# BenLangmead/bowtie2

Hardware: AMD Instinct MI355X
Metric: aligned reads/sec (whole node), 150 bp SE vs hg38-like synthetic genome (hg38 unavailable offline), large index (higher is better)
Workload: dtype u8/u64

## Files before the change

bowtie2_amd/csrc/bt2g_align.hpp:

```cpp
#ifndef BT2G_ALIGN_HPP_
#define BT2G_ALIGN_HPP_

#include "bt2g_device.hpp"
#include "../../include/bt2g.h"

namespace bt2g {

#ifdef BT2G_CLASS_MAX_LEN
constexpr int kMaxLen      = BT2G_CLASS_MAX_LEN;
constexpr int kMaxOffs     = BT2G_CLASS_MAX_OFFS;
#else
constexpr int kMaxLen      = 512;
constexpr int kMaxOffs     = 64;
#endif
constexpr int kMaxMm1      = 1024;
constexpr int kMaxRanges   = 2 * kMaxOffs;
constexpr int kMaxSat2     = 4096;
#ifdef BT2G_CLASS_MAX_EDITS
constexpr int kMaxEdits    = BT2G_CLASS_MAX_EDITS;
#else
constexpr int kMaxEdits    = 200;
#endif
#ifdef BT2G_CLASS_MAX_WALK_EDITS
constexpr int kMaxWalkEdits = BT2G_CLASS_MAX_WALK_EDITS;
// ... 219 lines not shown
	uint64_t srow_joff[kMaxSatpos];
	SatPos   sp_view;
	uint32_t lists[kListArena];
	double   masses[kMaxSat2];
	uint8_t  elim[kMaxSat2];
	struct ExtRange { uint32_t off, len, sz; } ex_fw[kMaxRanges * 2], ex_rc[kMaxRanges * 2];
	ExtRange ex_fw2[kMaxRanges * 2], ex_rc2[kMaxRanges * 2];
	DiagIval diags[kMaxDiags];
	int64_t  red_dmin[kMaxAlns], red_dmax[kMaxAlns];
	AlnRes   alns[kMaxAlns];
	BtCand   cands[kMaxCands];
	uint32_t cand_hist[2 * (kMaxLocalScore + 1)];
	uint32_t cand_done[2][kMaxCandDone];
	AlnRes   res;
	BtCand   cands2[kMaxCands];
	BtCand   cands_tmp[kMaxCands];
#ifndef BT2G_NO_PAIRS
	struct MateSave {
		uint32_t len;
		EEHit    exact[2];
		uint32_t n_mm1; uint64_t mm1_elt;
		uint32_t num_offs, nonz_tot, nonz_fw, nonz_rc, n_sranges; uint64_t num_elts;
		uint32_t off_idx2off[kMaxOffs];
		HotHit   hits[2][kMaxOffs];
		EEHit    mm1[kMaxMm1];
		SeedRange sranges[kMaxSat2];
	} ms[2];
	AlnRes   alns_u[2][kMaxAlnsU];
	AlnRes   alns_p[2][kMaxAlns];
	int64_t  redu_dmin[2][kMaxAlnsU], redu_dmax[2][kMaxAlnsU];
	AlnRes   red_anchor[kMaxRedAnchor];
	int64_t  reda_dmin[kMaxRedAnchor], reda_dmax[kMaxRedAnchor];
	AlnRes   ores;
	uint32_t mate_streaks[kMaxSatpos];
#endif
};

BT2_HD uint32_t dp_R(uint32_t rows) {
	const uint32_t r = (rows + 63) / 64;
	return (kMaxLen > 512 && r > 8) ? (r + 7) & ~7u : r;
}
BT2_HD uint64_t dp_cell(uint32_t R, uint32_t i, uint32_t j) {
	const uint32_t l = i / R, r = i % R;
	const uint64_t t = (uint64_t)j + l;
	return (t * R + r) * 64 + l;
}
BT2_HD uint32_t dp_RB(uint32_t rows) { const uint32_t r = (rows + 127) / 128; return r <= 4 ? r : r <= 8 ? 8u : 16u; }
BT2_HD uint64_t dp_cell_pk(uint32_t RB, uint32_t i, uint32_t j) {
	const uint32_t k = i / RB, r = i % RB;
	const uint64_t t = (uint64_t)j + k;
	return (t * RB + r) * 128 + (k >> 6) * 64 + (k & 63);
}
BT2_HD uint64_t dp_pk_cells(uint32_t rows, uint32_t cols) { const uint32_t RB = dp_RB(rows); return ((uint64_t)cols + (rows + RB - 1) / RB) * RB * 128; }


struct DpScratch {
	BT2_G uint32_t* mat;
	BT2_G uint16_t* masks;
	BT2_G uint32_t* pmask;
	BT2_G uint32_t* epoch;
	uint32_t  pmask_words;
};
enum { PB_HD = 1, PB_HE = 2, PB_HF = 4, PB_EO = 8, PB_EE = 16, PB_FO = 32, PB_FE = 64 };
constexpr uint32_t kEpochShift = 13, kEpochMax = (1u << 19) - 1;
constexpr uint32_t kPredTile = 64;
struct EeBand { int32_t lo; uint32_t nd; };
BT2_HD bool ee_band(int rfgapo, int rfgape, uint32_t rows, uint32_t cols, int64_t minsc, EeBand& b) {
	const int64_t budget = -minsc;
	if (budget < 0 || rows == 0 || cols == 0) return false;
	int64_t g;
	if (budget < rfgapo) g = 0; else if (rfgape <= 0) g = rows; else g = (budget - rfgapo) / rfgape + 1;
	if (g > (int64_t)rows - 1) g = (int64_t)rows - 1;
	int64_t dhi = (int64_t)cols - (int64_t)rows + g;
	if (dhi > (int64_t)cols - 1) dhi = (int64_t)cols - 1;
	if (dhi < -g) return false;
	b.lo = (int32_t)g; b.nd = (uint32_t)(dhi + g + 1);
	return true;
}
BT2_HD uint32_t ee_band_rp(uint32_t nd) {
	const uint32_t need = (nd + 127) / 128;
	return need <= 4 ? need : need <= 6 ? 6u : need <= 8 ? 8u : need <= 12 ? 12u : need <= 16 ? 16u : 0u;
}
BT2_HD uint64_t pred_idx(int32_t lo, uint32_t w, uint32_t i, uint32_t j) { return (uint64_t)i * w + (uint32_t)((int32_t)j - (int32_t)i + lo); }
BT2_HD uint64_t pred_at(int32_t lo, uint32_t w, uint32_t i, uint32_t j) { return w ? pred_idx(lo, w, i, j) : dp_cell_pk((uint32_t)lo, i, j); }
BT2_HD uint64_t pred_cells(uint32_t rows, uint32_t cols) { uint32_t rp = ee_band_rp(rows + cols); if (rp == 0) rp = 16; return (uint64_t)rows * rp * 128; }

struct AlState {
	BT2_G Work* wp;
	BT2_HD Work* wp_generic() const { return (Work*)wp; }
	DpScratch dp;
	Rng       rnd;
	int64_t   minsc;
	uint32_t  ridx;
	bool      ext_pre;
	const BT2_G uint32_t* pre_ext_cur;
	const BT2_G uint64_t* pre_joff_cur;
	uint32_t  pf_steps, pf_tiles;
	uint64_t  pf_tile_t;
	uint8_t   m_nofw, m_norc;
	const BT2_G uint8_t* pe_seq[2];
	const BT2_G uint8_t* pe_qual[2];
	uint32_t  pe_len[2];
	ReadParams pe_rp[2];
	int64_t   pe_minsc[2];
	DpScratch dp_main, dp_opp;
	BT2_G BtCand* cands_cur;
	uint32_t  pe_streak;
	uint32_t  pe_pair;
	uint32_t  n_emit;
	int32_t   emit_vmax;
	uint32_t  emit_on;
	uint32_t  max_cols;
	uint32_t  rf_at, ned_at;
	uint32_t  rt_at, rt_bytes, rt_cur;
	uint32_t  wide_cells;
	uint32_t  dyn_bytes;
	uint32_t  fill_rows_done, fill_lastsol, fill_sat8;
};

BT2_HD uint32_t dp_cols_for(const AlignParams& P) { return P.max_dp_cols > kMaxCols ? (uint32_t)(P.max_dp_cols < kMaxColsWide ? P.max_dp_cols : kMaxColsWide) : (uint32_t)kMaxCols; }
BT2_HD uint32_t hot_tail_off(uint32_t max_cols) { return (max_cols + 8 + 15) & ~15u; }
BT2_HD uint32_t hot_tail_bytes(uint32_t max_cols, bool local = true) {
	uint32_t b = (max_cols + 8) * 2;
	if (b < (uint32_t)(kMaxEdits * sizeof(Edit))) b = (uint32_t)(kMaxEdits * sizeof(Edit));
	if (kMaxWalkEdits > kMaxEdits && local && b < (uint32_t)(kMaxWalkEdits * sizeof(Edit))) b = (uint32_t)(kMaxWalkEdits * sizeof(Edit));
	if (local && b < kRadixCntBytes) b = kRadixCntBytes;
	return hot_tail_off(max_cols) + ((b + 15) & ~15u);
}

BT2_HD int comp4(int c) { return c < 4 ? 3 - c : 4; }
BT2_HD int imin(int a, int b) { return a < b ? a : b; }
BT2_HD int imax(int a, int b) { return a > b ? a : b; }
BT2_HD int subs0(int a, int b) { const int r = a - b; return r < 0 ? 0 : r; }

BT2_HD uint8_t code2chr(int c) { return (uint8_t)((0x4E54474341ull >> (8 * (c > 4 ? 4 : c))) & 0xff); }

template <typename SP> BT2_HD int mm_penalty(const SP& P, int q) {
	if (P.mm_type == 3) {
		const int qq = q < 40 ? q : 40;
		const float frac = (float)qq / 40.0f;
		return P.mm_min + (int)(frac * (float)(P.mm_max - P.mm_min));
	}
	if (P.mm_type == 2) return q < 5 ? 0 : (q < 15 ? 10 : (q < 25 ? 20 : 30));
	return P.mm_max;
}

template <typename SP> BT2_HD int sc_score(const SP& P, int rdc, int refm, int q) {
	if (q < 0) q = 0;
	if (q > 255) q = 255;
	if (rdc > 3 || refm > 15) return -P.n_pen;
	if (refm & (1 << rdc)) return P.match_bonus;
	return -mm_penalty(P, q);
}
template <typename SP> BT2_HD int sc_mm(const SP& P, int rdc, int refm, int q) {
	if (q < 0) q = 0;
	if (q > 255) q = 255;
	return (rdc > 3 || refm > 15) ? P.n_pen : mm_penalty(P, q);
}

BT2_HD int max_read_gaps(const AlignParams& P, int64_t minsc, uint32_t rdlen) {
	int64_t sc = (int64_t)rdlen * P.match_bonus;
	bool first = true;
	int num = 0;
	while (sc >= minsc) {
		if (first) { first = false; sc -= P.rdgapo; } else sc -= P.rdgape;
		num++;
	}
	return num - 1;
// ... 33 lines not shown
```

bowtie2_amd/csrc/bt2g_align_kernel.hip:

```cpp
#include <hip/hip_runtime.h>
#include <cstddef>
#include <cstdio>
#include <cstdlib>
#include <new>
#include <type_traits>
#include "bt2g_align_core.hpp"
#include "bt2g_local_pk.hpp"
#include "bt2g_align_kernel.hpp"

namespace bt2g {

__shared__ HotWork g_hot;
__shared__ AlignParams g_P;
__shared__ ReadParams g_rp;
__shared__ PreComp g_pre;
__shared__ AlState g_st;
extern __shared__ __attribute__((aligned(16))) uint8_t g_tail[];
typedef __attribute__((address_space(3))) uint8_t lds_byte;
__device__ __forceinline__ uint32_t lds_addr_of_tail() { return (uint32_t)reinterpret_cast<uintptr_t>((lds_byte*)g_tail); }
__device__ __forceinline__ uint8_t* lds_at(uint32_t a) { return (uint8_t*)reinterpret_cast<lds_byte*>((uintptr_t)(uint32_t)__builtin_amdgcn_readfirstlane((int)a)); }
__device__ __forceinline__ uint8_t* dev_rf() { return lds_at(g_st.rf_at); }
__device__ __forceinline__ int16_t* dev_lastrow() { return reinterpret_cast<int16_t*>(lds_at(g_st.ned_at)); }
__device__ __forceinline__ Edit* dev_ned() { return reinterpret_cast<Edit*>(lds_at(g_st.ned_at)); }
__device__ __forceinline__ uint32_t* dev_rt() { return reinterpret_cast<uint32_t*>(lds_at(g_st.rt_at)); }
alignas(16) __shared__ unsigned char g_ix_raw[sizeof(DevIndex<uint64_t>) > sizeof(DevIndex<uint32_t>) ? sizeof(DevIndex<uint64_t>) : sizeof(DevIndex<uint32_t>)];

__device__ __forceinline__ void wave_fence() { __builtin_amdgcn_fence(__ATOMIC_SEQ_CST, "workgroup"); }

typedef unsigned short u16x2 __attribute__((ext_vector_type(2)));
__device__ __forceinline__ u16x2 p_make(unsigned short lo, unsigned short hi) { u16x2 v; v.x = lo; v.y = hi; return v; }
__device__ __forceinline__ u16x2 p_splat(int v) { return p_make((unsigned short)v, (unsigned short)v); }
__device__ __forceinline__ u16x2 p_subs(u16x2 a, u16x2 b) { return __builtin_elementwise_sub_sat(a, b); }
__device__ __forceinline__ u16x2 p_max(u16x2 a, u16x2 b) { return __builtin_elementwise_max(a, b); }
__device__ __forceinline__ u16x2 p_min(u16x2 a, u16x2 b) { return __builtin_elementwise_min(a, b); }
__device__ __forceinline__ unsigned short s_subs(unsigned short a, unsigned short b) { return __builtin_elementwise_sub_sat(a, b); }
__device__ __forceinline__ unsigned short s_max(unsigned short a, unsigned short b) { return a > b ? a : b; }
__device__ __forceinline__ uint32_t umax32(uint32_t a, uint32_t b) { return a > b ? a : b; }
__device__ __forceinline__ uint32_t p_bits(u16x2 v) { return __builtin_bit_cast(uint32_t, v); }
__device__ __forceinline__ u16x2 p_from(uint32_t v) { return __builtin_bit_cast(u16x2, v); }
__device__ __forceinline__ u16x2 p_ne(u16x2 a, u16x2 b) { return p_from(pk::nz(p_bits(a ^ b))); }
__device__ __forceinline__ uint32_t shift_in(uint32_t lo, uint32_t hi) { return __builtin_amdgcn_alignbit(hi, lo, 16); }
template <int CTRL, int ROW_MASK>
__device__ __forceinline__ uint32_t dpp0(uint32_t v) { return (uint32_t)__builtin_amdgcn_update_dpp(0, (int)v, CTRL, ROW_MASK, 0xf, true); }
constexpr int kDppRowShr = 0x110, kDppWaveShl1 = 0x130, kDppWaveShr1 = 0x138, kDppBcast15 = 0x142, kDppBcast31 = 0x143;

template <int RP, bool PRED, bool W16>
__device__ __forceinline__ int fill_ee_u8_band(const AlignParams& P, bool fw, uint32_t rows, uint32_t cols, int lo, int thr, uint8_t* __restrict__ pm, uint32_t& rows_done) {
	constexpr uint32_t kBias = W16 ? 0xffffu : 0xffu;
	constexpr int kLastLo = W16 ? -32768 : -0xff;
	rows_done = rows;
	constexpr int N2 = 2 * RP;
	constexpr uint32_t W = 128u * RP;
	const int lane = threadIdx.x & 63;
	const int dd0 = lane * N2;
	const int j00 = dd0 - lo;
	uint32_t refS[RP];
	u16x2 Hp[RP], Fp[RP];
#pragma unroll
	for (int k = 0; k < RP; k++) {
		uint32_t sel = 0, h = 0;
#pragma unroll
		for (int hh = 0; hh < 2; hh++) {
			const int j = j00 + 2 * k + hh;
			const bool real = (uint32_t)j < cols;
			const uint32_t code = real ? (uint32_t)__builtin_ctz((uint32_t)dev_rf()[real ? j : 0] | 16u) : 4u;
			sel |= (code | 0x0c00u) << (16 * hh);
			h |= (real ? kBias : 0u) << (16 * hh);
		}
		refS[k] = sel; Hp[k] = p_from(h); Fp[k] = p_splat(0);
	}
	if (PRED) for (uint32_t j = (uint32_t)lane; j < cols; j += 64) dev_lastrow()[j] = (int16_t)kLastLo;
	const int rdgape = __builtin_amdgcn_readfirstlane(P.rdgape), rdgapo = __builtin_amdgcn_readfirstlane(P.rdgapo), gapbar = __builtin_amdgcn_readfirstlane(P.gapbar);
	const u16x2 rdoP = p_splat(rdgapo), rfoP = p_splat(__builtin_amdgcn_readfirstlane(P.rfgapo)), rfeP = p_splat(__builtin_amdgcn_readfirstlane(P.rfgape));
	uint32_t npen_word = (uint32_t)__builtin_amdgcn_readfirstlane(P.n_pen) & 0xffu;
	uint32_t k7f = 0x007f007fu;
	asm("" : "+v"(npen_word), "+v"(k7f));
	const int jin63 = 64 * N2 - lo;
	auto cap = [](uint32_t v) -> unsigned short { constexpr uint32_t m = W16 ? 0xffffu : 1023u; return (unsigned short)(v > m ? m : v); };
	const uint32_t D = (uint32_t)N2 * (uint32_t)rdgape;
	const uint32_t lD = (uint32_t)lane * D, lDprev = lane ? lD - D : 0u;
	u16x2 decP[RP];
#pragma unroll
	for (int k = 0; k < RP; k++) decP[k] = p_make(cap((uint32_t)(2 * k) * (uint32_t)rdgape), cap((uint32_t)(2 * k + 1) * (uint32_t)rdgape));
	u16x2 HP[RP];
#pragma unroll
	for (int k = 0; k < RP; k++) HP[k] = p_splat(0);
	for (uint32_t c0 = 0; c0 < rows; c0 += 64) {
		uint32_t tab = 0;
		{
			const uint32_t ri = c0 + (uint32_t)lane;
			if (ri < rows) {
				const int c = rd_char(g_hot, g_hot.len, fw, ri);
				const int q = rd_qual(g_hot, g_hot.len, fw, ri) - 33;
				const uint32_t mm = (uint32_t)(c > 3 ? P.n_pen : mm_penalty(P, q < 0 ? 0 : q)) & 0xffu;
				tab = mm * 0x01010101u;
				if (c <= 3) tab &= ~(0xffu << (8 * c));
			}
		}
		uint32_t chq;
		{
			int jc = jin63 + (int)c0 + lane; jc = jc < 0 ? 0 : jc; if (jc > (int)cols) jc = (int)cols;
			chq = (uint32_t)__builtin_ctz((uint32_t)dev_rf()[jc] | 16u) | 0x0c00u;
		}
		const uint32_t nrow = (uint32_t)__builtin_amdgcn_readfirstlane((int)(rows - c0 < 64u ? rows - c0 : 64u));
		for (uint32_t ii = 0; ii < nrow; ii++) {
			const uint32_t i = c0 + ii;
			const uint32_t T1 = (uint32_t)__builtin_amdgcn_readlane((int)tab, (int)ii);
			const bool bar = (int)i < gapbar || (int)(rows - i - 1) < gapbar;
			const bool nof = bar || i == 0;
			const uint32_t nxtH = dpp0<kDppWaveShl1, 0xf>(p_bits(Hp[0])), nxtF = dpp0<kDppWaveShl1, 0xf>(p_bits(Fp[0]));
			u16x2 penP[RP], HupP[RP], FupP[RP], fP[RP], HdP[RP];
#pragma unroll
			for (int k = 0; k < RP; k++) {
				penP[k] = p_from(__builtin_amdgcn_perm(npen_word, T1, refS[k]));
				HupP[k] = p_from(shift_in(p_bits(Hp[k]), k + 1 < RP ? p_bits(Hp[k + 1 < RP ? k + 1 : 0]) : nxtH));
				FupP[k] = p_from(shift_in(p_bits(Fp[k]), k + 1 < RP ? p_bits(Fp[k + 1 < RP ? k + 1 : 0]) : nxtF));
				fP[k] = nof ? p_splat(0) : p_max(p_subs(FupP[k], rfeP), p_subs(HupP[k], rfoP));
				HdP[k] = p_max(p_subs(Hp[k], penP[k]), fP[k]);
			}
			u16x2 EP[RP];
			if (!bar) {
				unsigned short e0[N2];
				unsigned short carry = 0;
#pragma unroll
				for (int c = 0; c < N2; c++) {
					const u16x2 u = p_subs(HdP[c >> 1], rdoP);
					e0[c] = carry;
					carry = s_max(s_subs(carry, (unsigned short)rdgape), (c & 1) ? u.y : u.x);
				}
				uint32_t Y = (uint32_t)carry + lD;
				Y = umax32(Y, dpp0<kDppRowShr + 1, 0xf>(Y));
				Y = umax32(Y, dpp0<kDppRowShr + 2, 0xf>(Y));
				Y = umax32(Y, dpp0<kDppRowShr + 4, 0xf>(Y));
				Y = umax32(Y, dpp0<kDppRowShr + 8, 0xf>(Y));
				Y = umax32(Y, dpp0<kDppBcast15, 0xa>(Y));
				Y = umax32(Y, dpp0<kDppBcast31, 0xc>(Y));
				const uint32_t Pprev = dpp0<kDppWaveShr1, 0xf>(Y);
				const u16x2 einP = p_splat((int)(Pprev - lDprev));
#pragma unroll
				for (int k = 0; k < RP; k++) EP[k] = p_max(p_make(e0[2 * k], e0[2 * k + 1]), p_subs(einP, decP[k]));
			} else {
#pragma unroll
				for (int k = 0; k < RP; k++) EP[k] = p_splat(0);
			}
#pragma unroll
			for (int k = 0; k < RP; k++) HP[k] = p_max(HdP[k], EP[k]);
			if (PRED) {
				const uint32_t prvH = dpp0<kDppWaveShr1, 0xf>(p_bits(HP[RP - 1])), prvE = dpp0<kDppWaveShr1, 0xf>(p_bits(EP[RP - 1]));
				const u16x2 rdeP = p_splat(rdgape);
				const uint32_t nogap = bar ? (uint32_t)(PB_HE | PB_HF) * 0x10001u : 0u;
				BT2_G uint8_t* rowp = (BT2_G uint8_t*)pm + (uint64_t)i * W + (uint32_t)dd0;
#pragma unroll
				for (int k = 0; k < RP; k++) {
					const u16x2 hlP = p_from(shift_in(k > 0 ? p_bits(HP[k > 0 ? k - 1 : 0]) : prvH, p_bits(HP[k])));
					const u16x2 elP = p_from(shift_in(k > 0 ? p_bits(EP[k > 0 ? k - 1 : 0]) : prvE, p_bits(EP[k])));
					const u16x2 h = HP[k], e = EP[k], f = fP[k];
					uint32_t n = p_bits(p_ne(f + rfeP, FupP[k]));
					n = pk::shl1_or(n, p_bits(p_ne(f + rfoP, HupP[k])));
					n = pk::shl1_or(n, p_bits(p_ne(e + rdeP, elP)));
					n = pk::shl1_or(n, p_bits(p_ne(e + rdoP, hlP)));
					n = pk::shl1_or(n, p_bits(p_ne(h, f)));
					n = pk::shl1_or(n, p_bits(p_ne(h, e)));
					n = pk::shl1_or(n, p_bits(p_ne(h + penP[k], Hp[k])));
					const uint32_t c = (n | nogap) ^ k7f;
					*reinterpret_cast<BT2_G uint16_t*>(rowp + 2 * k) = (uint16_t)__builtin_amdgcn_perm(0u, c, 0x0c0c0200u);
				}
			}
#pragma unroll
			for (int k = 0; k < RP; k++) { Hp[k] = HP[k]; Fp[k] = fP[k]; }
			if (!PRED && (i & 3u) == 3u) {
				u16x2 m = HP[0];
#pragma unroll
				for (int k = 1; k < RP; k++) m = p_max(m, HP[k]);
				if (!__any((int)s_max(m.x, m.y) >= thr)) { rows_done = i + 1; return 0; }
			}
			{
				uint32_t newel = dpp0<kDppWaveShl1, 0xf>(refS[0]);
				{ const int sq = __builtin_amdgcn_readlane((int)chq, (int)ii); asm("v_writelane_b32 %0, %1, 63" : "+v"(newel) : "s"(sq)); }
#pragma unroll
				for (int k = 0; k < RP; k++) refS[k] = shift_in(refS[k], k + 1 < RP ? refS[k + 1 < RP ? k + 1 : 0] : newel);
			}
		}
	}
	int best = 0;
	const int jl0 = (int)rows - 1 + j00;
#pragma unroll
	for (int k = 0; k < RP; k++) {
#pragma unroll
		for (int hh = 0; hh < 2; hh++) {
			const int j = jl0 + 2 * k + hh;
			const int h = hh ? (int)HP[k].y : (int)HP[k].x;
			if ((uint32_t)j < cols) { best = imax(best, h); if (PRED) dev_lastrow()[j] = (int16_t)imax(h - (int)kBias, kLastLo); }
		}
	}
#pragma unroll
	for (int s = 32; s > 0; s >>= 1) best = imax(best, __shfl_xor(best, s));
	return best;
}

constexpr int kLo = -32768;
__device__ __forceinline__ int subs16(int a, int b) { const int v = a - b; return v < kLo ? kLo : v; }

template <int R>
__device__ __forceinline__ int fill_ee_i16_wave(const AlignParams& P, bool fw, uint32_t rows, uint32_t cols,
                                               uint64_t* __restrict__ scratch) {
	const int lane = threadIdx.x & 63;
	const uint32_t nlanes = (rows + R - 1) / R;
	int rdc[R], mmp[R], veto[R];
#pragma unroll
	for (int r = 0; r < R; r++) {
		const uint32_t i = (uint32_t)lane * R + r;
		const bool valid = i < rows;
		rdc[r] = valid ? rd_char(g_hot, g_hot.len, fw, i) : 4;
		const int q = valid ? rd_qual(g_hot, g_hot.len, fw, i) - 33 : 0;
		mmp[r] = mm_penalty(P, q < 0 ? 0 : q);
		veto[r] = (valid && ((int)i < P.gapbar || (int)(rows - i - 1) < P.gapbar)) ? 1 : 0;
	}
	int Hprev[R], Eprev[R];
#pragma unroll
	for (int r = 0; r < R; r++) { Hprev[r] = kLo; Eprev[r] = kLo; }
	int myHlast = kLo, myFlast = kLo, upHdiag = kLo, refm = 0, best = kLo;
	const uint32_t steps = cols + nlanes - 1;
	const bool lane_has_last = ((rows - 1) / R) == (uint32_t)lane;
	const int last_r = (int)((rows - 1) % R);
	for (uint32_t t = 0; t < steps; t++) {
		const int upH = __shfl_up(myHlast, 1);
		const int upF = __shfl_up(myFlast, 1);
		int upRef = __shfl_up(refm, 1);
		if (lane == 0) upRef = (t < cols) ? dev_rf()[t] : 16;
		refm = upRef;
		const int j = (int)t - lane;
		const bool active = j >= 0 && j < (int)cols && (uint32_t)lane < nlanes;
		int refc = 4;
		if (refm & 1) refc = 0; else if (refm & 2) refc = 1; else if (refm & 4) refc = 2; else if (refm & 8) refc = 3;
		int hdiag = (lane == 0) ? 0x7fff : (j == 0 ? kLo : upHdiag);
		int fin_h = upH, fin_f = upF;
		int Hnew[R], Enew[R], Fnew[R];
#pragma unroll
		for (int r = 0; r < R; r++) {
			int pen;
			if (rdc[r] > 3 || refc > 3) pen = P.n_pen; else pen = (rdc[r] == refc) ? -P.match_bonus : mmp[r];
			const int e = (j == 0) ? kLo : imax(subs16(Eprev[r], P.rdgape), veto[r] ? kLo : subs16(Hprev[r], P.rdgapo));
			int f;
			if (lane == 0 && r == 0) f = kLo;
			else f = veto[r] ? kLo : imax(subs16(fin_f, P.rfgape), subs16(fin_h, P.rfgapo));
			const int h = imax(imax(subs16(hdiag, pen), e), f);
			Hnew[r] = h; Enew[r] = e; Fnew[r] = f;
			hdiag = Hprev[r];
			fin_h = h; fin_f = f;
		}
		if (active) {
			uint64_t* base = scratch + ((uint64_t)t * R) * 64 + lane;
#pragma unroll
			for (int r = 0; r < R; r++) base[r * 64] = (uint64_t)(uint16_t)Hnew[r] | ((uint64_t)(uint16_t)Enew[r] << 16) | ((uint64_t)(uint16_t)Fnew[r] << 32);
#pragma unroll
			for (int r = 0; r < R; r++) { Hprev[r] = Hnew[r]; Eprev[r] = Enew[r]; }
			if (lane_has_last) best = imax(best, Hnew[last_r]);
		}
		upHdiag = upH;
		if (active) { myHlast = Hnew[R - 1]; myFlast = Fnew[R - 1]; }
	}
	return __shfl(best, (int)((rows - 1) / R));
}

// ... 499 lines not shown
		for (int q = 0; q < K; q++) {
			if (__ballot((idx >> 6) == (uint32_t)q) == 0ull) continue;
			const uint32_t g = (uint32_t)__builtin_amdgcn_ds_bpermute((int)((idx & 63u) << 2), (int)v[q]);
			if ((idx >> 6) == (uint32_t)q) r = g;
		}
		return r;
	}
	static __device__ __forceinline__ void flush_samp_rows(BT2_G SampRow* dst, uint32_t lo, uint32_t hi, uint32_t src, uint32_t cnt) {
		const uint32_t l = threadIdx.x & 63;
		if (l < cnt) { SampRow r; r.topf = ((uint64_t)hi << 32) | lo; r.src = src; r.done = 0; gst(dst + l, r); }
	}
	template <typename TOff>
	static __device__ __forceinline__ void resolve_rows(const DevEbwt<TOff>& e, const SampRow* rows, uint32_t n, uint64_t* out) {
		wave_fence();
		const uint32_t lane = threadIdx.x & 63;
		if (lane < n) {
			uint32_t steps = 0;
			const TOff joff = bt2g::get_offset(e, (TOff)rows[lane].topf, steps);
			out[lane] = joff_pack((uint64_t)joff, steps);
		}
		wave_fence();
	}
	static __device__ __forceinline__ bool contains_u32(const uint32_t* p, uint32_t n, uint32_t v) {
		wave_fence();
		const uint32_t lane = threadIdx.x & 63;
		for (uint32_t base = 0; base < n; base += 64) {
			const uint32_t i = base + lane;
			if (__ballot(i < n && gld(p + (i < n ? i : 0)) == v)) return true;
		}
		return false;
	}
	static __device__ __attribute__((noinline)) void unseen_list(const uint32_t* seen_, uint32_t nseen_, uint32_t n_, uint32_t* out_) {
		wave_fence();
		const uint32_t* seen = uni_ptr(seen_); uint32_t* out = uni_ptr(out_);
		const uint32_t nseen = uni(nseen_), n = uni(n_);
		const uint32_t lane = threadIdx.x & 63;
		uint32_t count = 0;
		for (uint32_t p0 = 0; p0 < n; p0 += 2048) {
			uint32_t bm = 0;
			for (uint32_t base = 0; base < nseen; base += 64) {
				const uint32_t mine = base + lane < nseen ? gld(seen + base + lane) : 0xffffffffu;
				const uint32_t cnt = nseen - base < 64u ? nseen - base : 64u;
				for (uint32_t t = 0; t < cnt; t++) {
					const uint32_t v = (uint32_t)__builtin_amdgcn_readlane((int)mine, (int)t) - p0;
					if (v < 2048u && (v >> 5) == lane) bm |= 1u << (v & 31);
				}
			}
			const uint32_t pend = n - p0 < 2048u ? n - p0 : 2048u;
			for (uint32_t b = 0; b < pend; b += 64) {
				const uint32_t j = b + lane;
				const uint32_t word = (uint32_t)__shfl((int)bm, (int)(j >> 5));
				const bool unseen = j < pend && !((word >> (j & 31)) & 1u);
				const unsigned long long m = __ballot(unseen);
				if (unseen) gst(out + count + (uint32_t)__popcll(m & ((1ull << lane) - 1ull)), p0 + j);
				count += (uint32_t)__popcll(m);
			}
		}
		wave_fence();
	}
	static __device__ __forceinline__ void iota_u32(uint32_t* p, uint32_t n) {
		wave_fence();
		for (uint32_t i = threadIdx.x & 63; i < n; i += 64) gst(p + i, i);
		wave_fence();
	}
	static __device__ __forceinline__ void copy_words(void* dst, const void* src, uint32_t nwords) {
		wave_fence();
		const uint32_t* s = reinterpret_cast<const uint32_t*>(src);
		uint32_t* d = reinterpret_cast<uint32_t*>(dst);
		for (uint32_t i = threadIdx.x & 63; i < nwords; i += 64) gst(d + i, gld(s + i));
		wave_fence();
	}
	static __device__ __forceinline__ void set_epoch(uint32_t* p, uint32_t e) { if ((threadIdx.x & 63) == 0) *p = e; wave_fence(); }
	static __device__ __forceinline__ void bt_tile_pred(const DpScratch& dp, int32_t band_lo, uint32_t band_w, uint32_t row, uint32_t col, uint32_t epoch, uint32_t dir,
	                                                    uint32_t& pr, uint32_t& mk) {
		wave_fence();
		const uint32_t d = threadIdx.x & 63;
		uint32_t p = 0, m = 0;
		const uint32_t dr = dir == 1 ? 0u : d, dc = dir == 2 ? 0u : d;
		const uint32_t dd = (uint32_t)((int32_t)col - (int32_t)row + band_lo) + dr - dc;
		const bool ok = dr <= row && dc <= col && (band_w == 0u || dd < band_w);
		if (uni(g_st.rt_cur)) {
			if (ok) {
				const uint32_t r = row - dr, bit = r * band_w + dd;
				p = gld(reinterpret_cast<const uint8_t*>(dp.mat) + (uint64_t)r * band_w + dd);
				m = (dev_rt()[bit >> 5] >> (bit & 31u)) & 1u;
			}
		} else if (ok) {
			const uint64_t idx = pred_at(band_lo, band_w, row - dr, col - dc);
			p = gld(reinterpret_cast<const uint8_t*>(dp.mat) + idx);
			const uint32_t w = gld(dp.pmask + idx);
			m = (w >> kEpochShift) == epoch ? (w & 1u) : 0u;
		}
		pr = p; mk = m;
	}
	static __device__ __forceinline__ bool marks_batchable() { return true; }
	static __device__ __forceinline__ void pred_tile8(const DpScratch& dp, int32_t band_lo, uint32_t band_w, uint32_t epoch, uint32_t row, uint32_t col, uint32_t dir, uint32_t flag,
	                                                  uint32_t& plo, uint32_t& phi, uint32_t& mk) {
		wave_fence();
		const uint8_t* pm = reinterpret_cast<const uint8_t*>(dp.mat);
		const bool chip = uni(g_st.rt_cur) != 0u;
		uint32_t pb[8], mw[8];
#pragma unroll
		for (uint32_t i = 0; i < 8; i++) {
			const uint32_t r = row - (dir == 1u ? 0u : i), c = col - (dir == 2u ? 0u : i);
			const uint32_t dd = (uint32_t)((int32_t)c - (int32_t)r + band_lo);
			const bool ok = flag && (int32_t)r >= 0 && (int32_t)c >= 0 && dd < band_w;
			const uint32_t bit = r * band_w + dd;
			pb[i] = ok ? (uint32_t)gld(pm + (uint64_t)r * band_w + dd) : 0u;
			if (chip) mw[i] = ok ? (dev_rt()[bit >> 5] >> (bit & 31u)) & 1u : 0u;
			else { const uint32_t w = ok ? gld(dp.pmask + (uint64_t)r * band_w + dd) : 0u; mw[i] = (w >> kEpochShift) == epoch ? (w & 1u) : 0u; }
		}
		plo = pb[0] | (pb[1] << 8) | (pb[2] << 16) | (pb[3] << 24);
		phi = pb[4] | (pb[5] << 8) | (pb[6] << 16) | (pb[7] << 24);
		mk = mw[0] | (mw[1] << 1) | (mw[2] << 2) | (mw[3] << 3) | (mw[4] << 4) | (mw[5] << 5) | (mw[6] << 6) | (mw[7] << 7);
	}
	static __device__ __forceinline__ uint32_t marks_of_cells(const DpScratch& dp, int32_t band_lo, uint32_t band_w, uint32_t epoch, uint32_t r, uint32_t c, uint32_t flag) {
		wave_fence();
		const uint32_t dd = (uint32_t)((int32_t)c - (int32_t)r + band_lo);
		const bool ok = flag && (int32_t)r >= 0 && (int32_t)c >= 0 && dd < band_w;
		const uint32_t bit = r * band_w + dd;
		if (uni(g_st.rt_cur)) return ok ? (dev_rt()[bit >> 5] >> (bit & 31u)) & 1u : 0u;
		const uint32_t w = ok ? gld(dp.pmask + (uint64_t)r * band_w + dd) : 0u;
		return (w >> kEpochShift) == epoch ? (w & 1u) : 0u;
	}
	static __device__ __forceinline__ void mark_cells(const DpScratch& dp, int32_t band_lo, uint32_t band_w, uint32_t epoch, uint32_t r, uint32_t c, uint32_t flag) {
		const uint32_t dd = (uint32_t)((int32_t)c - (int32_t)r + band_lo);
		const bool ok = flag && (int32_t)r >= 0 && (int32_t)c >= 0 && dd < band_w;
		const uint32_t bit = r * band_w + dd;
		if (uni(g_st.rt_cur)) { if (ok) __hip_atomic_fetch_or(dev_rt() + (bit >> 5), 1u << (bit & 31u), __ATOMIC_RELAXED, __HIP_MEMORY_SCOPE_WAVEFRONT); }
		else if (ok) gst(dp.pmask + (uint64_t)r * band_w + dd, 1u | (epoch << kEpochShift));
		wave_fence();
	}
	static __device__ __forceinline__ void rt_mark(const DpScratch& dp, int32_t band_lo, uint32_t band_w, uint32_t epoch, uint32_t row, uint32_t col) {
		if (uni(g_st.rt_cur)) {
			const uint32_t bit = row * band_w + (uint32_t)((int32_t)col - (int32_t)row + band_lo);
			if ((threadIdx.x & 63) == 0) __hip_atomic_fetch_or(dev_rt() + (bit >> 5), 1u << (bit & 31u), __ATOMIC_RELAXED, __HIP_MEMORY_SCOPE_WAVEFRONT);
		} else gst(dp.pmask + pred_at(band_lo, band_w, row, col), 1u | (epoch << kEpochShift));
	}
	static __device__ __forceinline__ void rt_mark_lane(const DpScratch& dp, int32_t band_lo, uint32_t band_w, uint32_t epoch, uint32_t r, uint32_t c) {
		if (uni(g_st.rt_cur)) {
			const uint32_t bit = r * band_w + (uint32_t)((int32_t)c - (int32_t)r + band_lo);
			__hip_atomic_fetch_or(dev_rt() + (bit >> 5), 1u << (bit & 31u), __ATOMIC_RELAXED, __HIP_MEMORY_SCOPE_WAVEFRONT);
		} else gst(dp.pmask + pred_at(band_lo, band_w, r, c), 1u | (epoch << kEpochShift));
	}
	static __device__ __forceinline__ void rt_begin(const DpScratch& dp, uint32_t rows, bool band) {
		wave_fence();
		const uint32_t w = band ? uni(gld(dp.epoch + 2)) : 0u;
		const uint32_t rt_bytes = uni(g_st.rt_bytes);
		const bool on = w != 0u && rows * (w >> 3) <= rt_bytes;
		if (on) {
			uint4* q = reinterpret_cast<uint4*>(dev_rt());
			const uint32_t n16 = (rows * (w >> 3) + 15u) >> 4;
			for (uint32_t i = threadIdx.x & 63; i < n16; i += 64) q[i] = make_uint4(0, 0, 0, 0);
		}
		if ((threadIdx.x & 63) == 0) g_st.rt_cur = on ? 1u : 0u;
		wave_fence();
	}
	static __device__ __forceinline__ void load_seed_hits(const bt2g_seed_hit* src_fw, const bt2g_seed_hit* src_rc, uint32_t nseeds, bool skip_fw, bool skip_rc) {
		for (int fwi = 0; fwi < 2; fwi++) {
			const bt2g_seed_hit* src = fwi == 0 ? src_fw : src_rc;
			const bool skip = fwi == 0 ? skip_fw : skip_rc;
			for (uint32_t i = threadIdx.x & 63; i < nseeds; i += 64) {
				HotHit h; h.topf = h.topb = 0; h.size = h.esize = 0;
				if (!skip) {
					const uint64_t topf = gld(&src[i].topf), botf = gld(&src[i].botf);
					if (botf > topf) { h.topf = topf; h.topb = gld(&src[i].topb); h.size = h.esize = (uint32_t)(botf - topf); }
				}
				g_hot.hits[fwi][i] = h;
				g_hot.sorted[fwi][i] = 0;
			}
		}
	}
	static __device__ __forceinline__ uint64_t seed_key(bool fw, uint32_t depth, uint32_t L, bool& ok) {
		const uint32_t k = threadIdx.x & 63;
		uint64_t part = 0;
		bool bad = false;
		if (k < L) {
			const int ch = fw ? (int)g_hot.seq[depth + k] : comp4(g_hot.seq[depth + L - 1 - k]);
			bad = ch > 3;
			part = (uint64_t)(ch & 3) << (2 * (L - 1 - k));
		}
		ok = __ballot(bad) == 0ull;
		uint32_t lo = (uint32_t)part, hi = (uint32_t)(part >> 32);
#pragma unroll
		for (int s = 32; s > 0; s >>= 1) { lo |= (uint32_t)__shfl_xor((int)lo, s); hi |= (uint32_t)__shfl_xor((int)hi, s); }
		return ((uint64_t)hi << 32) | lo;
	}
	static __device__ __forceinline__ uint32_t find_key(const uint64_t* keys, const uint8_t* lens, uint32_t n, uint64_t key, uint8_t len) {
		const uint32_t lane = threadIdx.x & 63;
		for (uint32_t base = 0; base < n; base += 64) {
			const uint32_t i = base + lane;
// ... 682 lines not shown
	};
	if (P.paired) {
#ifdef BT2G_NO_PAIRS
		return hipErrorInvalidValue;
#else
		const uint32_t extra = spare(reinterpret_cast<const void*>(&k_align_pairs<TOff>), tail);
		hipLaunchKernelGGL(k_align_pairs<TOff>, dim3(n_waves), dim3(64), tail + extra, st, ix, P, rd, d_rparams, d_results, result_stride,
		                   d_arena, arena_stride, mat_bytes, mask_bytes, pmask_bytes, d_next, d_prof, pre, max_read_len, max_cols, 0u, extra);
#endif
	} else {
		uint32_t rt_bytes = 0;
		hipFuncAttributes fa{};
		static const bool rt_off = getenv("BT2G_RT_LDS") && atoi(getenv("BT2G_RT_LDS")) == 0;
		if (!rt_off && P.match_bonus == 0 && lds_per_wave != 0 && hipFuncGetAttributes(&fa, reinterpret_cast<const void*>(&k_align_reads<TOff>)) == hipSuccess) {
			const uint64_t used = (uint64_t)fa.sharedSizeBytes + tail;
			const uint32_t want = ((max_read_len ? max_read_len : 1u) * 16u + 15u) & ~15u;
			if (used + want <= lds_per_wave) rt_bytes = want;
		}
		const uint32_t extra = spare(reinterpret_cast<const void*>(&k_align_reads<TOff>), tail + rt_bytes);
		static const bool dbg_occ = getenv("BT2G_DEBUG_OCC") != nullptr;
		if (dbg_occ) {
			int nb = 0;
			(void)hipOccupancyMaxActiveBlocksPerMultiprocessor(&nb, reinterpret_cast<const void*>(&k_align_reads<TOff>), 64, tail + rt_bytes + extra);
			fprintf(stderr, "[bt2g] k_align_reads: %d waves per CU resident (LDS %u static + %u tail + %u marks + %u spare; budget %u per wave), %u waves launched\n",
			        nb, (unsigned)fa.sharedSizeBytes, tail, rt_bytes, extra, lds_per_wave, n_waves);
		}
		hipLaunchKernelGGL(k_align_reads<TOff>, dim3(n_waves), dim3(64), tail + rt_bytes + extra, st, ix, P, rd, d_rparams, d_results, result_stride,
		                   d_arena, arena_stride, mat_bytes, mask_bytes, pmask_bytes, d_next, d_prof, pre, max_read_len, max_cols, rt_bytes, extra);
	}
	return hipGetLastError();
}

__global__ void __launch_bounds__(64) __attribute__((amdgpu_waves_per_eu(BT2G_WAVES_PER_EU, BT2G_WAVES_PER_EU), amdgpu_num_vgpr(BT2G_NUM_VGPR)))
k_dp_fill(AlignParams P, const bt2g_dp_problem* __restrict__ probs, uint32_t n, const uint8_t* __restrict__ d_rd, const uint8_t* __restrict__ d_qu,
          const uint8_t* __restrict__ d_rf, uint8_t* __restrict__ d_out, uint8_t* __restrict__ scratch, uint64_t scratch_stride,
          uint64_t mat_bytes, uint64_t mask_bytes, uint64_t pmask_bytes, uint32_t max_cols) {
	const uint32_t lane = threadIdx.x & 63;
	g_P = P;
	g_st.max_cols = max_cols; g_st.rf_at = lds_addr_of_tail(); g_st.ned_at = g_st.rf_at + hot_tail_off(max_cols);
	g_st.rt_at = 0; g_st.rt_bytes = 0; g_st.rt_cur = 0; g_st.dyn_bytes = 0; g_st.wide_cells = 0;
	DpScratch dp;
	carve_scratch(dp, scratch + (uint64_t)blockIdx.x * scratch_stride, mat_bytes, mask_bytes, pmask_bytes);
	g_st.dp = dp; g_st.wp = (BT2_G Work*)scratch; g_st.emit_on = 0;
	wave_fence();
	for (uint32_t p = blockIdx.x; p < n; p += gridDim.x) {
		const bt2g_dp_problem pr = probs[p];
		const uint32_t rows = pr.rows, cols = pr.cols;
		BT2_G bt2g_dp_out* out = (BT2_G bt2g_dp_out*)(d_out + pr.out_off);
		wave_fence();
		g_hot.len = rows;
		for (uint32_t i = lane; i < rows; i += 64) { g_hot.seq[i] = d_rd[pr.rd_off + i]; g_hot.qual[i] = d_qu[pr.rd_off + i]; }
		for (uint32_t j = lane; j < cols + 1; j += 64) dev_rf()[j] = d_rf[pr.rf_off + j];
		g_hot.n_dp_cells_score = g_hot.n_dp_cells_full = g_hot.n_dp_pass = 0;
		wave_fence();
		int64_t best;
		uint32_t lastsolcol = 0, sat8 = 0;
		if (pr.kind == BT2G_DP_LOCAL) best = DevPlat::dp_fill_local(g_P, *g_st.wp_generic(), true, rows, cols, (uint32_t*)dp.mat, (int64_t)pr.minsc, lastsolcol, sat8);
		else {
			const bool band_form = pr.kind == BT2G_DP_EE_U8 || pr.kind == BT2G_DP_EE_I16_BAND;
			if ((threadIdx.x & 63) == 0) g_st.wide_cells = pr.kind == BT2G_DP_EE_I16 ? 1u : 0u;
			wave_fence();
			best = (pr.kind == BT2G_DP_EE_I16_BAND && !DevPlat::ee_wide_band(rows, cols, (int64_t)pr.minsc)) ? INT64_MIN
			     : DevPlat::dp_fill_ee(g_P, *g_st.wp_generic(), true, rows, cols, dp, pr.kind != BT2G_DP_EE_U8, (int64_t)pr.minsc);
			(void)band_form;
		}
		wave_fence();
		const bool band_kind = pr.kind == BT2G_DP_EE_U8 || pr.kind == BT2G_DP_EE_I16_BAND;
		const bool has_mat = !band_kind || (best != INT64_MIN && best >= (int64_t)pr.minsc);
		const int32_t band_lo = (int32_t)dp.epoch[1];
		const uint32_t band_w = dp.epoch[2];
		if (lane == 0) {
			out->best = best; out->lastsolcol = lastsolcol; out->sat8 = sat8; out->pad = 0;
			out->band_lo = band_kind && has_mat ? band_lo : 0; out->band_w = band_kind && has_mat ? band_w : 0;
			out->has_matrix = has_mat ? 1u : 0u;
		}
		BT2_G uint8_t* body = (BT2_G uint8_t*)(d_out + pr.out_off + sizeof(bt2g_dp_out));
		if (band_kind) {
			const uint32_t c4 = (cols + 3u) & ~3u;
			BT2_G int16_t* lr = (BT2_G int16_t*)body;
			for (uint32_t j = lane; j < c4; j += 64) lr[j] = (has_mat && j < cols) ? dev_lastrow()[j] : (int16_t)(pr.kind == BT2G_DP_EE_U8 ? -0xff : -32768);
			if (has_mat) {
				BT2_G uint8_t* pm = body + (uint64_t)c4 * 2;
				const BT2_G uint8_t* src = (const BT2_G uint8_t*)dp.mat;
				for (uint64_t k = lane; k < (uint64_t)rows * band_w; k += 64) pm[k] = src[k];
			}
		} else if (pr.kind == BT2G_DP_LOCAL) {
			const uint32_t RB = dp_RB(rows);
			const BT2_G uint8_t* src = (const BT2_G uint8_t*)dp.mat;
			const uint64_t ncell = (uint64_t)rows * cols;
			for (uint64_t k = lane; k < ncell; k += 64) body[k] = src[dp_cell_pk(RB, (uint32_t)(k / cols), (uint32_t)(k % cols))];
		} else {
			const uint32_t R = dp_R(rows);
			const BT2_G uint64_t* m64 = (const BT2_G uint64_t*)dp.mat;
			BT2_G int32_t* H = (BT2_G int32_t*)body;
			const uint64_t ncell = (uint64_t)rows * cols;
			for (uint64_t k = lane; k < ncell; k += 64) {
				const uint32_t i = (uint32_t)(k / cols), j = (uint32_t)(k % cols);
				const uint64_t c = m64[dp_cell(R, i, j)];
				const uint32_t h = (uint32_t)(c & 0xffff), e = (uint32_t)((c >> 16) & 0xffff), f = (uint32_t)((c >> 32) & 0xffff);
				if (pr.kind == BT2G_DP_EE_I16) { H[k] = (int32_t)(int16_t)h; H[ncell + k] = (int32_t)(int16_t)e; H[2 * ncell + k] = (int32_t)(int16_t)f; }
				else { H[k] = (int32_t)h; H[ncell + k] = (int32_t)e; H[2 * ncell + k] = (int32_t)f; }
			}
		}
		wave_fence();
	}
}

hipError_t launch_dp_fill(const AlignParams& P, const bt2g_dp_problem* d_probs, uint32_t n, const uint8_t* d_rd, const uint8_t* d_qu, const uint8_t* d_rf,
                          uint8_t* d_out, uint8_t* d_scratch, uint64_t scratch_stride, uint64_t mat_bytes, uint64_t mask_bytes, uint64_t pmask_bytes,
                          uint32_t n_waves, uint32_t max_cols, hipStream_t st) {
	if (n == 0) return hipSuccess;
	hipLaunchKernelGGL(k_dp_fill, dim3(n < n_waves ? n : n_waves), dim3(64), hot_tail_bytes(max_cols), st, P, d_probs, n, d_rd, d_qu, d_rf, d_out, d_scratch, scratch_stride, mat_bytes, mask_bytes, pmask_bytes, max_cols);
	return hipGetLastError();
}

void align_scratch_sizes(uint32_t max_len, bool paired, uint32_t maxhalf, uint32_t max_cols, uint64_t& mat_bytes, uint64_t& mask_bytes, uint64_t& pmask_bytes, uint64_t& arena_stride) {
	const uint32_t rows = max_len ? max_len : 1;
	const uint32_t R = dp_R(rows);
	uint32_t cols = paired ? max_cols + 4 : rows + 4 * maxhalf + 1 + 4;
	if (cols > max_cols + 4) cols = max_cols + 4;
	const uint32_t lanes = (rows + R - 1) / R;
	mat_bytes = (((uint64_t)cols + lanes) * R * 64 * 8 + 255) & ~(uint64_t)255;
	const uint64_t pred_bytes = (pred_cells(rows, cols) + 255) & ~(uint64_t)255;
	if (pred_bytes > mat_bytes) mat_bytes = pred_bytes;
	mask_bytes = ((uint64_t)rows * cols * 2 + 255) & ~(uint64_t)255;
#ifdef BT2G_KCLASS_W5
	mat_bytes = pred_bytes; mask_bytes = 256;
#endif
	const uint64_t wf_cells = ((uint64_t)cols + 128) * dp_RB(rows) * 128;
	const uint64_t mask_cells = pred_cells(rows, cols) > wf_cells ? pred_cells(rows, cols) : wf_cells;
	pmask_bytes = 256 + ((mask_cells * 4 + 255) & ~(uint64_t)255);
	arena_stride = ((sizeof(Work) + 255) & ~(uint64_t)255) + (paired ? 2 : 1) * (mat_bytes + mask_bytes + pmask_bytes);
	arena_stride = (arena_stride + 4095) & ~(uint64_t)4095;
}

uint64_t align_work_bytes() { return sizeof(Work); }
uint32_t align_waves_per_cu() { return 4u * BT2G_WAVES_PER_EU; }

template hipError_t launch_align<uint32_t>(const DevIndex<uint32_t>&, const AlignParams&, const bt2g_reads&, const ReadParams*, uint8_t*, uint64_t, uint8_t*, uint64_t, uint64_t, uint64_t, uint64_t, uint32_t, unsigned int*, unsigned long long*, const PreComp&, uint32_t, uint32_t, uint32_t, hipStream_t);
template hipError_t launch_align<uint64_t>(const DevIndex<uint64_t>&, const AlignParams&, const bt2g_reads&, const ReadParams*, uint8_t*, uint64_t, uint8_t*, uint64_t, uint64_t, uint64_t, uint64_t, uint32_t, unsigned int*, unsigned long long*, const PreComp&, uint32_t, uint32_t, uint32_t, hipStream_t);

}

#define BT2G_CLASS_ENTRIES(PFX) \
extern "C" hipError_t PFX##_launch_align(int off_size, const void* ix, const bt2g_align_params* P, const bt2g_reads* rd, const bt2g_read_params* d_rparams, \
                                         uint8_t* d_results, uint64_t result_stride, uint8_t* d_arena, uint64_t arena_stride, \
                                         uint64_t mat_bytes, uint64_t mask_bytes, uint64_t pmask_bytes, uint32_t n_waves, unsigned int* d_next, unsigned long long* d_prof, \
                                         const void* pre, uint32_t max_read_len, uint32_t max_cols, uint32_t lds_per_wave, hipStream_t st) { \
	using namespace bt2g; \
	const PreComp& pc = *reinterpret_cast<const PreComp*>(pre); \
	return off_size == 4 \
		? launch_align(*reinterpret_cast<const DevIndex<uint32_t>*>(ix), *P, *rd, d_rparams, d_results, result_stride, d_arena, arena_stride, mat_bytes, mask_bytes, pmask_bytes, n_waves, d_next, d_prof, pc, max_read_len, max_cols, lds_per_wave, st) \
		: launch_align(*reinterpret_cast<const DevIndex<uint64_t>*>(ix), *P, *rd, d_rparams, d_results, result_stride, d_arena, arena_stride, mat_bytes, mask_bytes, pmask_bytes, n_waves, d_next, d_prof, pc, max_read_len, max_cols, lds_per_wave, st); \
} \
extern "C" uint32_t PFX##_waves_per_cu(void) { return bt2g::align_waves_per_cu(); } \
 \
extern "C" uint32_t PFX##_static_lds(void) { \
	hipFuncAttributes a32, a64; \
	if (hipFuncGetAttributes(&a32, reinterpret_cast<const void*>(&bt2g::k_align_reads<uint32_t>)) != hipSuccess) return 0xffffffffu; \
	if (hipFuncGetAttributes(&a64, reinterpret_cast<const void*>(&bt2g::k_align_reads<uint64_t>)) != hipSuccess) return 0xffffffffu; \
	return (uint32_t)(a32.sharedSizeBytes > a64.sharedSizeBytes ? a32.sharedSizeBytes : a64.sharedSizeBytes); \
} \
extern "C" uint64_t PFX##_work_bytes(void) { return bt2g::align_work_bytes(); } \
 \
extern "C" uint32_t PFX##_max_len(void) { return (uint32_t)bt2g::kMaxLen; } \
extern "C" uint32_t PFX##_max_offs(void) { return (uint32_t)bt2g::kMaxOffs; } \
extern "C" uint32_t PFX##_max_alns(void) { return (uint32_t)bt2g::kMaxAlns; } \
 \
extern "C" void PFX##_scratch_sizes(uint32_t max_len, int paired, uint32_t maxhalf, uint32_t max_cols, uint64_t* mat_bytes, uint64_t* mask_bytes, uint64_t* pmask_bytes, uint64_t* arena_stride) { \
	bt2g::align_scratch_sizes(max_len, paired != 0, maxhalf, max_cols, *mat_bytes, *mask_bytes, *pmask_bytes, *arena_stride); \
}
#ifdef BT2G_KCLASS_W5
BT2G_CLASS_ENTRIES(bt2g_w5)
#endif
#ifdef BT2G_KCLASS_BK
BT2G_CLASS_ENTRIES(bt2g_bk)
#endif
#ifdef BT2G_KCLASS_LR
BT2G_CLASS_ENTRIES(bt2g_lr)
#endif
```

Before: 6.447 million.

## Block predecessor matrix rows so each lane writes 16-byte vector stores

Changes the banded predecessor-matrix layout so several consecutive rows (RB = 8/4/2 depending on RP) are interleaved into 1 KiB blocks. Each lane accumulates its per-row codes in registers and issues one 16-byte store per block, replacing many 2-byte scattered stores during the DP fill. Readers in the traceback and debug-dump paths switch to the new blocked address function, and the scratch size rounds rows up to a multiple of 8. The cost is extra register shuffling per row, padding stores for partial blocks, and more complex indexing on the traceback loads.

Result: no change. 6.462 million, median of 3 (+0.2%).

```diff
diff --git a/bowtie2_amd/csrc/bt2g_align.hpp b/bowtie2_amd/csrc/bt2g_align.hpp
--- a/bowtie2_amd/csrc/bt2g_align.hpp
+++ b/bowtie2_amd/csrc/bt2g_align.hpp
@@ -325,8 +325,15 @@
 	return need <= 4 ? need : need <= 6 ? 6u : need <= 8 ? 8u : need <= 12 ? 12u : need <= 16 ? 16u : 0u;
 }
 BT2_HD uint64_t pred_idx(int32_t lo, uint32_t w, uint32_t i, uint32_t j) { return (uint64_t)i * w + (uint32_t)((int32_t)j - (int32_t)i + lo); }
+BT2_HD uint32_t pred_band_rb_log2(uint32_t w) { return w == 128u ? 3u : w == 256u ? 2u : w == 512u ? 1u : 0u; }
+BT2_HD uint64_t pred_band_at(uint32_t w, uint32_t i, uint32_t dd) {
+	const uint32_t rbs = pred_band_rb_log2(w), n2s = rbs ? 4u - rbs : 0u;
+	return (uint64_t)(i >> rbs) * (w << rbs) + ((dd >> n2s) << (n2s + rbs)) + ((i & ((1u << rbs) - 1u)) << n2s) + (dd & ((1u << n2s) - 1u));
+}
+BT2_HD uint64_t pred_band_bytes(uint32_t w, uint32_t rows) { return (uint64_t)((rows + 7u) & ~7u) * w; }
 BT2_HD uint64_t pred_at(int32_t lo, uint32_t w, uint32_t i, uint32_t j) { return w ? pred_idx(lo, w, i, j) : dp_cell_pk((uint32_t)lo, i, j); }
 BT2_HD uint64_t pred_cells(uint32_t rows, uint32_t cols) { uint32_t rp = ee_band_rp(rows + cols); if (rp == 0) rp = 16; return (uint64_t)rows * rp * 128; }
+BT2_HD uint64_t pred_band_cells(uint32_t rows, uint32_t cols) { uint32_t rp = ee_band_rp(rows + cols); if (rp == 0) rp = 16; return pred_band_bytes(rp * 128u, rows); }
 
 struct AlState {
 	BT2_G Work* wp;
diff --git a/bowtie2_amd/csrc/bt2g_align_kernel.hip b/bowtie2_amd/csrc/bt2g_align_kernel.hip
--- a/bowtie2_amd/csrc/bt2g_align_kernel.hip
+++ b/bowtie2_amd/csrc/bt2g_align_kernel.hip
@@ -85,6 +85,23 @@
 	u16x2 HP[RP];
 #pragma unroll
 	for (int k = 0; k < RP; k++) HP[k] = p_splat(0);
+	constexpr uint32_t RBS = RP == 1 ? 3u : RP == 2 ? 2u : RP == 4 ? 1u : 0u, RB = 1u << RBS;
+	uint32_t blk[4] = {0u, 0u, 0u, 0u};
+	auto blk_push = [&](const uint32_t* cb) {
+		if constexpr (RP == 1) {
+			blk[0] = shift_in(blk[0], blk[1]); blk[1] = shift_in(blk[1], blk[2]); blk[2] = shift_in(blk[2], blk[3]);
+			blk[3] = __builtin_amdgcn_perm(cb[0], blk[3], 0x06040302u);
+		} else if constexpr (RP == 2) {
+			blk[0] = blk[1]; blk[1] = blk[2]; blk[2] = blk[3]; blk[3] = __builtin_amdgcn_perm(cb[1], cb[0], 0x06040200u);
+		} else if constexpr (RP == 4) {
+			blk[0] = blk[2]; blk[1] = blk[3]; blk[2] = __builtin_amdgcn_perm(cb[1], cb[0], 0x06040200u); blk[3] = __builtin_amdgcn_perm(cb[3], cb[2], 0x06040200u);
+		}
+	};
+	auto blk_store = [&](uint32_t b) {
+		typedef uint32_t u32x4 __attribute__((ext_vector_type(4)));
+		u32x4 v; v.x = blk[0]; v.y = blk[1]; v.z = blk[2]; v.w = blk[3];
+		*reinterpret_cast<BT2_G u32x4*>((BT2_G uint8_t*)pm + ((uint64_t)b << 10) + ((uint32_t)lane << 4)) = v;
+	};
 	for (uint32_t c0 = 0; c0 < rows; c0 += 64) {
 		uint32_t tab = 0;
 		{
@@ -150,6 +167,7 @@
 				const u16x2 rdeP = p_splat(rdgape);
 				const uint32_t nogap = bar ? (uint32_t)(PB_HE | PB_HF) * 0x10001u : 0u;
 				BT2_G uint8_t* rowp = (BT2_G uint8_t*)pm + (uint64_t)i * W + (uint32_t)dd0;
+				uint32_t cb[RP];
 #pragma unroll
 				for (int k = 0; k < RP; k++) {
 					const u16x2 hlP = p_from(shift_in(k > 0 ? p_bits(HP[k > 0 ? k - 1 : 0]) : prvH, p_bits(HP[k])));
@@ -163,7 +181,12 @@
 					n = pk::shl1_or(n, p_bits(p_ne(h, e)));
 					n = pk::shl1_or(n, p_bits(p_ne(h + penP[k], Hp[k])));
 					const uint32_t c = (n | nogap) ^ k7f;
-					*reinterpret_cast<BT2_G uint16_t*>(rowp + 2 * k) = (uint16_t)__builtin_amdgcn_perm(0u, c, 0x0c0c0200u);
+					cb[k] = c;
+					if (RB == 1u) *reinterpret_cast<BT2_G uint16_t*>(rowp + 2 * k) = (uint16_t)__builtin_amdgcn_perm(0u, c, 0x0c0c0200u);
+				}
+				if (RB > 1u) {
+					blk_push(cb);
+					if ((ii & (RB - 1u)) == RB - 1u) blk_store(i >> RBS);
 				}
 			}
 #pragma unroll
@@ -180,6 +203,13 @@
 #pragma unroll
 				for (int k = 0; k < RP; k++) refS[k] = shift_in(refS[k], k + 1 < RP ? refS[k + 1 < RP ? k + 1 : 0] : newel);
 			}
+		}
+		if (PRED && RB > 1u && (nrow & (RB - 1u)) != 0u) {
+			uint32_t zero[RP];
+#pragma unroll
+			for (int k = 0; k < RP; k++) zero[k] = 0u;
+			for (uint32_t r = nrow & (RB - 1u); r < RB; r++) blk_push(zero);
+			blk_store((c0 + nrow - 1u) >> RBS);
 		}
 	}
 	int best = 0;
@@ -845,12 +875,12 @@
 		if (uni(g_st.rt_cur)) {
 			if (ok) {
 				const uint32_t r = row - dr, bit = r * band_w + dd;
-				p = gld(reinterpret_cast<const uint8_t*>(dp.mat) + (uint64_t)r * band_w + dd);
+				p = gld(reinterpret_cast<const uint8_t*>(dp.mat) + pred_band_at(band_w, r, dd));
 				m = (dev_rt()[bit >> 5] >> (bit & 31u)) & 1u;
 			}
 		} else if (ok) {
 			const uint64_t idx = pred_at(band_lo, band_w, row - dr, col - dc);
-			p = gld(reinterpret_cast<const uint8_t*>(dp.mat) + idx);
+			p = gld(reinterpret_cast<const uint8_t*>(dp.mat) + (band_w ? pred_band_at(band_w, row - dr, dd) : idx));
 			const uint32_t w = gld(dp.pmask + idx);
 			m = (w >> kEpochShift) == epoch ? (w & 1u) : 0u;
 		}
@@ -869,7 +899,7 @@
 			const uint32_t dd = (uint32_t)((int32_t)c - (int32_t)r + band_lo);
 			const bool ok = flag && (int32_t)r >= 0 && (int32_t)c >= 0 && dd < band_w;
 			const uint32_t bit = r * band_w + dd;
-			pb[i] = ok ? (uint32_t)gld(pm + (uint64_t)r * band_w + dd) : 0u;
+			pb[i] = ok ? (uint32_t)gld(pm + pred_band_at(band_w, r, dd)) : 0u;
 			if (chip) mw[i] = ok ? (dev_rt()[bit >> 5] >> (bit & 31u)) & 1u : 0u;
 			else { const uint32_t w = ok ? gld(dp.pmask + (uint64_t)r * band_w + dd) : 0u; mw[i] = (w >> kEpochShift) == epoch ? (w & 1u) : 0u; }
 		}
@@ -1718,7 +1748,7 @@
 			if (has_mat) {
 				BT2_G uint8_t* pm = body + (uint64_t)c4 * 2;
 				const BT2_G uint8_t* src = (const BT2_G uint8_t*)dp.mat;
-				for (uint64_t k = lane; k < (uint64_t)rows * band_w; k += 64) pm[k] = src[k];
+				for (uint64_t k = lane; k < (uint64_t)rows * band_w; k += 64) pm[k] = src[pred_band_at(band_w, (uint32_t)(k / band_w), (uint32_t)(k % band_w))];
 			}
 		} else if (pr.kind == BT2G_DP_LOCAL) {
 			const uint32_t RB = dp_RB(rows);
@@ -1757,7 +1787,7 @@
 	if (cols > max_cols + 4) cols = max_cols + 4;
 	const uint32_t lanes = (rows + R - 1) / R;
 	mat_bytes = (((uint64_t)cols + lanes) * R * 64 * 8 + 255) & ~(uint64_t)255;
-	const uint64_t pred_bytes = (pred_cells(rows, cols) + 255) & ~(uint64_t)255;
+	const uint64_t pred_bytes = (pred_band_cells(rows, cols) + 255) & ~(uint64_t)255;
 	if (pred_bytes > mat_bytes) mat_bytes = pred_bytes;
 	mask_bytes = ((uint64_t)rows * cols * 2 + 255) & ~(uint64_t)255;
 #ifdef BT2G_KCLASS_W5
```
